# sandialabs/implicit-sph

Hardware: AMD Instinct MI355X
Metric: pressure-Poisson solves/sec (3D TGV, 1M particles per GPU, GMRES(50)+block-Jacobi ILU(0), tol 1e-8) (higher is better)
Workload: dtype f64; 1 GPU; 3D Taylor-Green vortex, 100^3 particles per GPU, Wendland cut=2h (BASELINE configs[1]), state after one Lagrangian step (mode=advect); rows_per_gpu=1000000, global_rows=1000000, nnz_per_gpu=103845090, solver=FGMRES(50) DGKS tol 1e-8, right prec, precond=bjacobi-ilu0, atom_order=lexicographic, library_row_order=bricks, parallelism=domain bricks 1x1x1, RCCL halo + all-reduce, restarts=1, converged=1

## Files before the change

### implicit-sph_amd/csrc/core.hpp

```cpp
#pragma once
#include "common.hpp"
#include "order.hpp"
#include "sell.hpp"

namespace isph { struct HostStager; }

struct isph_neigh_layout {
  const void *nptr = nullptr;
  const int *nidx = nullptr, *colmap = nullptr;
  const void *order = nullptr;
  int n = -1, is_sorted = 0;
  isph::DevBuf<long long> off;
  isph::DevBuf<int> idx, len, sorted;
  void release() { off.release(); idx.release(); len.release(); sorted.release(); nptr = nullptr; nidx = colmap = nullptr; order = nullptr; n = -1; is_sorted = 0; }
};

struct isph_neigh_map {
  const int *rowsrc = nullptr, *idmap = nullptr, *colmap_key = nullptr;
  const int *colkey = nullptr;
  const void *order = nullptr;
};

struct isph_table_cache {
  int ntypes = -1, kernel = -1, dim = -1;
  std::vector<int> kind;
  std::vector<double> h, cutsq;
  isph::DevBuf<int> dkind;
  isph::DevBuf<double> dh, dcutsq, dhinv, dknorm, dkdnorm;
  void release() { dkind.release(); dh.release(); dcutsq.release(); dhinv.release(); dknorm.release(); dkdnorm.release(); ntypes = -1; }
};

struct isph_ctx {
  int device = 0;
  hipStream_t stream = nullptr;
  bool own_stream = false;
  int rank = 0, nranks = 1;
  ncclComm_t comm = nullptr;
  isph_host_transport host_tr = {nullptr, nullptr, nullptr};
  double *hsend = nullptr, *hrecv = nullptr;
  size_t hsend_cap = 0, hrecv_cap = 0;
  bool profile = false;
  int stat_reorth = 0;
  isph::DevBuf<double> partial;
  isph::DevBuf<double> dscal;
  double *hscal = nullptr;
  size_t hscal_cap = 0;
  isph::DevBuf<double> V, Z, wv, tv, rv, pv, nvec, xext, sendbuf, bdev, xdev;
  isph::DevBuf<double> bint, xint;
  isph::DevBuf<int> imask, imask2;
  std::vector<hipEvent_t> ev;
  std::vector<int> ev_class;
  size_t ev_used = 0;
  std::vector<hipEvent_t> hev;
  size_t hev_used = 0;
  hipEvent_t ev0 = nullptr, ev1 = nullptr;
  hipEvent_t ev_fetch = nullptr;
  std::vector<hipEvent_t> ev_ls;
  hipStream_t comm_stream = nullptr;
  hipEvent_t ev_pack = nullptr, ev_halo = nullptr;
  isph::DevBuf<double> xghost;
  isph::HostStager *stager = nullptr;
  bool neigh_hold = false;
  isph_neigh_layout neigh_cache[2];
  isph_table_cache tables;
  int ordering = 1;
  isph::OrderBox box;
  isph_neigh_map nmap;
  isph::RowOrderPtr held_order;
  const void *held_key[2] = {nullptr, nullptr};
};

namespace isph {
enum ProfClass { PROF_SPMV = 0, PROF_PREC_APPLY, PROF_MULTI_DOT, PROF_MULTI_AXPY_DOT, PROF_MULTI_AXPY_NORM, PROF_ILU_EXTRACT,
                 PROF_ILU_SCHEDULE, PROF_ILU_FACTOR, PROF_NCLASS };
struct ProfScope {
  isph_ctx *c;
  size_t slot = (size_t)-1;
  ProfScope(isph_ctx *ctx, int cls, hipStream_t st = nullptr) : c(ctx) {
    if (!c || !c->profile || (st && st != c->stream)) return;
    if (c->ev_used + 2 > c->ev.size()) {
      hipEvent_t a = nullptr, b = nullptr;
      if (hipEventCreate(&a) != hipSuccess || hipEventCreate(&b) != hipSuccess) return;
      c->ev.push_back(a); c->ev.push_back(b);
      c->ev_class.push_back(cls);
    }
    slot = c->ev_used;
    c->ev_class[slot / 2] = cls;
    c->ev_used += 2;
    (void)hipEventRecord(c->ev[slot], c->stream);
  }
  ~ProfScope() { end(); }
  void end() {
    if (slot != (size_t)-1) (void)hipEventRecord(c->ev[slot + 1], c->stream);
    slot = (size_t)-1;
  }
};
}

// ... 40 lines not shown
```

### implicit-sph_amd/csrc/krylov.hpp

```cpp
#pragma once
#include "common.hpp"

namespace isph {

constexpr int kDotBatch = 16;

__global__ __launch_bounds__(kBlock) void k_multi_dot_v2(int n, int nk, const double *__restrict__ V, long long ld,
                                                         const double *__restrict__ w, double *__restrict__ partial) {
  __shared__ double sred[kDotBatch + 1][4];
  const int wave = threadIdx.x >> 6, lane = threadIdx.x & 63;
  const long long stride = (long long)gridDim.x * kBlock, np = n >> 1;
  const long long p0 = (long long)blockIdx.x * kBlock + threadIdx.x;
  const double2 *__restrict__ w2 = reinterpret_cast<const double2 *>(w);
  for (int k0 = 0; k0 < nk || k0 == 0; k0 += kDotBatch) {
    const int nb = min(kDotBatch, nk - k0);
    const bool last = k0 + kDotBatch >= nk;
    double acc[kDotBatch];
#pragma unroll
    for (int u = 0; u < kDotBatch; ++u) acc[u] = 0.0;
    double ww = 0.0;
    const double *__restrict__ vb = V + (long long)k0 * ld;
    for (long long p = p0; p < np; p += stride) {
      const double2 wi = w2[p];
      if (last) ww = fma(wi.y, wi.y, fma(wi.x, wi.x, ww));
// ... 69 lines not shown
#pragma unroll
      for (int u = 0; u < kDotBatch; ++u)
        if (u < nb) acc[u] = fma(vb[(long long)u * ld + i], wi, acc[u]);
    }
#pragma unroll
    for (int u = 0; u < kDotBatch; ++u) {
      if (u < nb) {
        const double s = wave_sum(acc[u]);
        if (lane == 0) sred[u][wave] = s;
      }
    }
    if (last) {
      ww = wave_sum(ww);
      if (lane == 0) sred[kDotBatch][wave] = ww;
    }
    __syncthreads();
    if (threadIdx.x < nb)
      partial[(long long)(k0 + threadIdx.x) * gridDim.x + blockIdx.x] =
          (sred[threadIdx.x][0] + sred[threadIdx.x][1]) + (sred[threadIdx.x][2] + sred[threadIdx.x][3]);
    if (last && threadIdx.x == 0)
      partial[(long long)nk * gridDim.x + blockIdx.x] =
          (sred[kDotBatch][0] + sred[kDotBatch][1]) + (sred[kDotBatch][2] + sred[kDotBatch][3]);
    __syncthreads();
    if (last) break;
  }
}

__global__ __launch_bounds__(kBlock) void k_reduce_partials(int nk, int nblk, const double *__restrict__ partial,
                                                            double *__restrict__ out,
                                                            const double *__restrict__ flag = nullptr) {
  __shared__ double sw[4];
  const int k = blockIdx.x;
  if (k >= nk) return;
  if (flag && *flag == 0.0) {
    if (threadIdx.x == 0) out[k] = 0.0;
    return;
  }
  const double *__restrict__ p = partial + (long long)k * nblk;
  double s0 = 0.0, s1 = 0.0, s2 = 0.0, s3 = 0.0;
  int b = threadIdx.x;
  for (; b + 3 * kBlock < nblk; b += 4 * kBlock) {
    s0 += p[b];
    s1 += p[b + kBlock];
    s2 += p[b + 2 * kBlock];
    s3 += p[b + 3 * kBlock];
  }
  for (; b < nblk; b += kBlock) s0 += p[b];
  double s = wave_sum((s0 + s1) + (s2 + s3));
  if ((threadIdx.x & 63) == 0) sw[threadIdx.x >> 6] = s;
  __syncthreads();
  if (threadIdx.x == 0) out[k] = (sw[0] + sw[1]) + (sw[2] + sw[3]);
}

__global__ __launch_bounds__(kBlock) void k_multi_axpy_norm(int n, int nk, const double *__restrict__ V, long long ld,
                                                            const double *__restrict__ c, double *__restrict__ w,
                                                            double *__restrict__ partial,
                                                            const double *__restrict__ dec_old = nullptr,
                                                            const double *__restrict__ dec_dn = nullptr, int dec_force = 0,
                                                            double *__restrict__ dec_out = nullptr,
                                                            double *__restrict__ vnext = nullptr) {
  __shared__ double sw[4];
  __shared__ double sdec[2];
  bool second = true;
  double wfinal2 = 1.0;
  if (dec_old) {
    if (threadIdx.x == 0) {
      double old2 = *dec_old;
      if (dec_dn) old2 = fmax(old2 - dec_dn[0] * dec_dn[0], 0.0);
      const double ww_new = c[nk];
      const bool sec = dec_force || sqrt(ww_new) < M_SQRT1_2 * sqrt(old2);
      double s2 = 0.0;
      for (int k = 0; k < nk; ++k) s2 += c[k] * c[k];
      sdec[0] = sec ? 1.0 : 0.0;
      sdec[1] = sec ? fmax(ww_new - s2, 0.0) : ww_new;
      if (blockIdx.x == 0) { dec_out[0] = sdec[0]; dec_out[1] = sdec[1]; }
    }
    __syncthreads();
    second = sdec[0] != 0.0;
    wfinal2 = sdec[1];
  }
  if (!second && !vnext) return;
  double a = 1.0;
  if (vnext) a *= 1.0 / sqrt(wfinal2);
  double ww = 0.0;
  for (long long i = (long long)blockIdx.x * blockDim.x + threadIdx.x; i < n; i += (long long)gridDim.x * blockDim.x) {
    double s = w[i];
    if (second) {
      for (int k = 0; k < nk; ++k) s = fma(-c[k], V[(long long)k * ld + i], s);
      w[i] = s;
    }
    if (vnext) vnext[i] = a * s;
    ww = fma(s, s, ww);
  }
  ww = wave_sum(ww);
  if ((threadIdx.x & 63) == 0) sw[threadIdx.x >> 6] = ww;
  __syncthreads();
  if (threadIdx.x == 0) partial[blockIdx.x] = (sw[0] + sw[1]) + (sw[2] + sw[3]);
}

template <int NK>
__global__ __launch_bounds__(kBlock) void k_multi_axpy_dot(int n, int nk, const double *__restrict__ V, long long ld,
                                                           const double *__restrict__ c, double *__restrict__ w,
                                                           double *__restrict__ partial) {
  __shared__ double sred[NK + 1][4];
  __shared__ double sc[NK];
  const int wave = threadIdx.x >> 6, lane = threadIdx.x & 63;
  if (threadIdx.x < NK) sc[threadIdx.x] = threadIdx.x < nk ? c[threadIdx.x] : 0.0;
  __syncthreads();
  double acc[NK];
#pragma unroll
  for (int u = 0; u < NK; ++u) acc[u] = 0.0;
  double ww = 0.0;
  const long long stride = (long long)gridDim.x * kBlock;
  for (long long i = (long long)blockIdx.x * kBlock + threadIdx.x; i < n; i += stride) {
    double v[NK];
#pragma unroll
    for (int u = 0; u < NK; ++u) v[u] = u < nk ? V[(long long)u * ld + i] : 0.0;
    double s = w[i];
#pragma unroll
    for (int u = 0; u < NK; ++u) s = fma(-sc[u], v[u], s);
    w[i] = s;
    ww = fma(s, s, ww);
#pragma unroll
    for (int u = 0; u < NK; ++u) acc[u] = fma(v[u], s, acc[u]);
  }
#pragma unroll
  for (int u = 0; u < NK; ++u) {
    if (u < nk) {
      const double r = wave_sum(acc[u]);
      if (lane == 0) sred[u][wave] = r;
    }
  }
  ww = wave_sum(ww);
  if (lane == 0) sred[NK][wave] = ww;
  __syncthreads();
  if (threadIdx.x < nk)
    partial[(long long)threadIdx.x * gridDim.x + blockIdx.x] =
        (sred[threadIdx.x][0] + sred[threadIdx.x][1]) + (sred[threadIdx.x][2] + sred[threadIdx.x][3]);
  if (threadIdx.x == 0)
    partial[(long long)nk * gridDim.x + blockIdx.x] = (sred[NK][0] + sred[NK][1]) + (sred[NK][2] + sred[NK][3]);
}

__global__ void k_multi_axpy(int n, int nk, const double *__restrict__ Z, long long ld, const double *__restrict__ c,
                             double *__restrict__ x) {
  for (long long i = (long long)blockIdx.x * blockDim.x + threadIdx.x; i < n; i += (long long)gridDim.x * blockDim.x) {
    double s = x[i];
    for (int k = 0; k < nk; ++k) s = fma(c[k], Z[(long long)k * ld + i], s);
    x[i] = s;
  }
}

__global__ __launch_bounds__(kBlock) void k_dot2(int n, const double *__restrict__ a, const double *__restrict__ b,
                                                 const double *__restrict__ c, const double *__restrict__ d,
                                                 double *__restrict__ partial) {
  __shared__ double s0[4], s1[4];
  double p = 0.0, q = 0.0;
  for (long long i = (long long)blockIdx.x * blockDim.x + threadIdx.x; i < n; i += (long long)gridDim.x * blockDim.x) {
    p = fma(a[i], b[i], p);
    if (c) q = fma(c[i], d[i], q);
  }
  p = wave_sum(p);
  q = wave_sum(q);
  if ((threadIdx.x & 63) == 0) { s0[threadIdx.x >> 6] = p; s1[threadIdx.x >> 6] = q; }
  __syncthreads();
  if (threadIdx.x == 0) {
    partial[blockIdx.x] = (s0[0] + s0[1]) + (s0[2] + s0[3]);
    partial[gridDim.x + blockIdx.x] = (s1[0] + s1[1]) + (s1[2] + s1[3]);
  }
}

__global__ void k_scale_copy(int n, const double *__restrict__ x, double *__restrict__ y, double alpha,
                             const double *__restrict__ s, int inv_sqrt) {
  double a = alpha;
  if (s) a *= inv_sqrt ? 1.0 / sqrt(*s) : *s;
  for (long long i = (long long)blockIdx.x * blockDim.x + threadIdx.x; i < n; i += (long long)gridDim.x * blockDim.x)
    y[i] = a * x[i];
}

__global__ void k_axpy_dev(int n, double alpha, const double *__restrict__ s, const double *__restrict__ x,
                           double *__restrict__ y) {
  const double a = s ? alpha * (*s) : alpha;
  for (long long i = (long long)blockIdx.x * blockDim.x + threadIdx.x; i < n; i += (long long)gridDim.x * blockDim.x)
    y[i] = fma(a, x[i], y[i]);
}

__global__ void k_residual(int n, const double *__restrict__ b, double *__restrict__ r) {
  for (long long i = (long long)blockIdx.x * blockDim.x + threadIdx.x; i < n; i += (long long)gridDim.x * blockDim.x)
    r[i] = b[i] - r[i];
}

__global__ void k_cg_update_p(int n, const double *__restrict__ z, double *__restrict__ p,
                              const double *__restrict__ num, const double *__restrict__ den) {
  const double beta = *num / *den;
  for (long long i = (long long)blockIdx.x * blockDim.x + threadIdx.x; i < n; i += (long long)gridDim.x * blockDim.x)
    p[i] = fma(beta, p[i], z[i]);
}

__global__ __launch_bounds__(kBlock) void k_cg_update_xr(int n, const double *__restrict__ p,
                                                         const double *__restrict__ ap, double *__restrict__ x,
                                                         double *__restrict__ r, const double *__restrict__ num,
                                                         const double *__restrict__ den, double *__restrict__ partial) {
  __shared__ double sw[4];
  const double a = *num / *den;
  double rr = 0.0;
  for (long long i = (long long)blockIdx.x * blockDim.x + threadIdx.x; i < n; i += (long long)gridDim.x * blockDim.x) {
    x[i] = fma(a, p[i], x[i]);
    const double t = fma(-a, ap[i], r[i]);
    r[i] = t;
    rr = fma(t, t, rr);
  }
  rr = wave_sum(rr);
  if ((threadIdx.x & 63) == 0) sw[threadIdx.x >> 6] = rr;
  __syncthreads();
  if (threadIdx.x == 0) partial[blockIdx.x] = (sw[0] + sw[1]) + (sw[2] + sw[3]);
}

__global__ void k_mul_elem(int n, const double *__restrict__ a, const double *__restrict__ b, double *__restrict__ y) {
  for (long long i = (long long)blockIdx.x * blockDim.x + threadIdx.x; i < n; i += (long long)gridDim.x * blockDim.x)
    y[i] = a[i] * b[i];
}

__global__ void k_fill(int n, double *__restrict__ y, double v) {
  for (long long i = (long long)blockIdx.x * blockDim.x + threadIdx.x; i < n; i += (long long)gridDim.x * blockDim.x)
    y[i] = v;
}

__global__ void k_mask_to_double(int n, const int *__restrict__ m, double *__restrict__ y) {
  for (long long i = (long long)blockIdx.x * blockDim.x + threadIdx.x; i < n; i += (long long)gridDim.x * blockDim.x)
    y[i] = (double)m[i];
}

inline int stream_grid(long long n) {
  long long g = (n + kBlock - 1) / kBlock;
  if (g > kMaxRedBlocks) g = kMaxRedBlocks;
  if (g < 1) g = 1;
  return (int)g;
}

}
```

### implicit-sph_amd/csrc/solver.hpp

```cpp
#pragma once
#include <cmath>

#include "comm.hpp"
#include "core.hpp"
#include "krylov.hpp"

namespace isph {

int prec_apply_dev(isph_ctx *ctx, const isph_prec *M, const double *r, double *z);
int prec_apply_multi_dev(isph_ctx *ctx, const isph_prec *M, int K, const double *const *rs, double *const *zs);

inline int allreduce_inplace(isph_ctx *ctx, double *d, int count) {
  return comm_allreduce(ctx, d, count,  0, ctx->stream);
}

enum { SC_DOT = 0 , SC_Y = 64 , SC_MISC = 128, SC_COUNT = 160 };

constexpr int kMaxLockstep = 4;

inline int ensure_scalars(isph_ctx *ctx) {
  ISPH_CHECK(ctx->dscal.reserve(SC_COUNT * kMaxLockstep));
  ISPH_CHECK(ctx->partial.reserve((size_t)kMaxRedBlocks * 66));
  if (ctx->hscal_cap < (size_t)SC_COUNT * kMaxLockstep) {
    if (ctx->hscal) (void)hipHostFree(ctx->hscal);
    ISPH_CHECK_HIP(hipHostMalloc((void **)&ctx->hscal, (size_t)SC_COUNT * kMaxLockstep * sizeof(double)));
    ctx->hscal_cap = (size_t)SC_COUNT * kMaxLockstep;
  }
  return ISPH_SUCCESS;
}

inline int fetch_scalars(isph_ctx *ctx, int first, int count) {
  ISPH_CHECK_HIP(hipMemcpyAsync(ctx->hscal + first, ctx->dscal.p + first, sizeof(double) * (size_t)count,
                                hipMemcpyDeviceToHost, ctx->stream));
  ISPH_CHECK_HIP(hipStreamSynchronize(ctx->stream));
  return ISPH_SUCCESS;
}

__global__ void k_gather(int n, const int *__restrict__ idx, const double *__restrict__ x, double *__restrict__ out) {
  for (int i = blockIdx.x * blockDim.x + threadIdx.x; i < n; i += gridDim.x * blockDim.x) out[i] = x[idx[i]];
}

inline int halo_begin(isph_ctx *ctx, const isph_mat *A, const double *x, hipEvent_t *hev = nullptr) {
  ISPH_REQUIRE(comm_active(ctx) && ctx->comm_stream,
               "a matrix with a halo needs a context made by isph_ctx_create_dist or isph_ctx_create_hostcomm");
  const Sell &S = A->S;
  const isph_halo &H = A->halo;
  ISPH_REQUIRE(H.nrecv == S.ncol - S.nrow, "matrix has ghost columns but no matching halo plan");
  ISPH_REQUIRE(H.n_int + H.n_bnd == S.nslices, "halo plan without the interior/boundary slice lists");
  ISPH_CHECK(ctx->xghost.reserve((size_t)(H.nrecv > 0 ? H.nrecv : 1)));
  ISPH_CHECK(ctx->sendbuf.reserve((size_t)(H.nsend > 0 ? H.nsend : 1)));
  if (H.nsend > 0)
    hipLaunchKernelGGL(k_gather, dim3(stream_grid(H.nsend)), dim3(kBlock), 0, ctx->stream, H.nsend, H.send_idx.p, x,
                       ctx->sendbuf.p);
  ISPH_CHECK_HIP(hipEventRecord(ctx->ev_pack, ctx->stream));
  if (hev) ISPH_CHECK_HIP(hipEventRecord(hev[0], ctx->stream));
  ISPH_CHECK_HIP(hipStreamWaitEvent(ctx->comm_stream, ctx->ev_pack, 0));
  ISPH_CHECK(comm_exchange(ctx, H, ctx->sendbuf.p, ctx->xghost.p, 1, false, ctx->comm_stream));
  ISPH_CHECK_HIP(hipEventRecord(ctx->ev_halo, ctx->comm_stream));
  if (hev) ISPH_CHECK_HIP(hipEventRecord(hev[1], ctx->comm_stream));
  return ISPH_SUCCESS;
}

inline bool sell_cols16(isph_ctx *ctx, const Sell &S) {
  if (S.c16_state != 0) return S.c16_state > 0;
  S.c16_state = -1;
  if (S.nslices == 0 || S.stored == 0) return false;
  DevTmp<int> flag;
  if (flag.reserve(1) != ISPH_SUCCESS || S.col16.reserve((size_t)S.stored) != ISPH_SUCCESS ||
      S.wtab.reserve((size_t)S.nslices * 64) != ISPH_SUCCESS) { flag.release(); return false; }
  int h = 0;
  if (hipMemsetAsync(flag.p, 0, sizeof(int), ctx->stream) == hipSuccess) {
    hipLaunchKernelGGL(k_sell_compress_cols, dim3((S.nslices + 3) / 4), dim3(kBlock), 0, ctx->stream, 0, S.nslices,
                       (const long long *)S.slice_off.p, (const int *)S.col.p, S.col16.p, S.wtab.p, flag.p);
    if (hipMemcpyAsync(&h, flag.p, sizeof(int), hipMemcpyDeviceToHost, ctx->stream) == hipSuccess &&
        hipStreamSynchronize(ctx->stream) == hipSuccess && hipGetLastError() == hipSuccess && h == 0)
      S.c16_state = 1;
  }
  flag.release();
// ... 111 lines not shown
          if (!first)
            hipLaunchKernelGGL(k_axpy_dev, dim3(stream_grid(nloc)), dim3(kBlock), 0, ctx->stream, nloc, 1.0,
                               (const double *)nullptr, (const double *)tmp, yi);
          first = false;
        }
        if (first) ISPH_CHECK_HIP(hipMemsetAsync(yi, 0, sizeof(double) * (size_t)nloc, ctx->stream));
      }
      return ISPH_SUCCESS;
    }
    ISPH_CHECK(spmv_dev(ctx, A, x, y, nvec));
    if (nvec)
      hipLaunchKernelGGL(k_axpy_dev, dim3(stream_grid(n)), dim3(kBlock), 0, ctx->stream, n, -1.0,
                         ctx->dscal.p + SC_MISC, nvec, y);
    return ISPH_SUCCESS;
  }
  int prec(const double *r, double *z) const {
    if (!M) {
      ISPH_CHECK_HIP(hipMemcpyAsync(z, r, sizeof(double) * (size_t)n, hipMemcpyDeviceToDevice, ctx->stream));
      return ISPH_SUCCESS;
    }
    if (blk) {
      const double *rs[4];
      double *zs[4];
      for (int i = 0; i < dim && i < 4; ++i) { rs[i] = r + (size_t)i * nloc; zs[i] = z + (size_t)i * nloc; }
      return prec_apply_multi_dev(ctx, M, dim, rs, zs);
    }
    return prec_apply_dev(ctx, M, r, z);
  }
};

inline int dot_dev(isph_ctx *ctx, int n, const double *a, const double *b, const double *c, const double *d, int slot) {
  const int g = stream_grid(n);
  hipLaunchKernelGGL(k_dot2, dim3(g), dim3(kBlock), 0, ctx->stream, n, a, b, c, d, ctx->partial.p);
  hipLaunchKernelGGL(k_reduce_partials, dim3(2), dim3(kBlock), 0, ctx->stream, 2, g, ctx->partial.p, ctx->dscal.p + slot);
  return allreduce_inplace(ctx, ctx->dscal.p + slot, 2);
}

inline int project_dev(isph_ctx *ctx, int n, const double *nvec, double *v) {
  ISPH_CHECK(dot_dev(ctx, n, v, nvec, nullptr, nullptr, SC_MISC + 2));
  hipLaunchKernelGGL(k_axpy_dev, dim3(stream_grid(n)), dim3(kBlock), 0, ctx->stream, n, -1.0, ctx->dscal.p + SC_MISC + 2,
                     nvec, v);
  return ISPH_SUCCESS;
}

inline int cgs_pass(isph_ctx *ctx, int n, int nk, const double *V, long long ld, double *w) {
  int g = stream_grid(n);
  if (g > 1024) g = 1024;
  ISPH_CHECK(ctx->partial.reserve((size_t)(nk + 2) * kMaxRedBlocks > (size_t)kMaxRedBlocks * 66 ? (size_t)(nk + 2) * kMaxRedBlocks : (size_t)kMaxRedBlocks * 66));
  hipLaunchKernelGGL((k_multi_dot<1>), dim3(g), dim3(kBlock), 0, ctx->stream, n, nk, V, ld, w, ctx->partial.p);
  hipLaunchKernelGGL(k_reduce_partials, dim3(nk + 1), dim3(kBlock), 0, ctx->stream, nk + 1, g, ctx->partial.p,
                     ctx->dscal.p + SC_DOT);
  ISPH_CHECK(allreduce_inplace(ctx, ctx->dscal.p + SC_DOT, nk + 1));
  const int g2 = stream_grid(n);
  hipLaunchKernelGGL(k_multi_axpy_norm, dim3(g2), dim3(kBlock), 0, ctx->stream, n, nk, V, ld, ctx->dscal.p + SC_DOT, w,
                     ctx->partial.p);
  hipLaunchKernelGGL(k_reduce_partials, dim3(1), dim3(kBlock), 0, ctx->stream, 1, g2, ctx->partial.p,
                     ctx->dscal.p + SC_DOT + nk + 1);
  ISPH_CHECK(allreduce_inplace(ctx, ctx->dscal.p + SC_DOT + nk + 1, 1));
  ISPH_CHECK_HIP(hipGetLastError());
  return fetch_scalars(ctx, SC_DOT, nk + 2);
}

enum { SC_ORTHO = SC_MISC + 20 };
inline int ortho_enqueue(isph_ctx *ctx, int n, int nk, const double *V, long long ld, double *w, int ortho, double *vnext,
                         bool deflate = false, int mb = 0) {
  int g = stream_grid(n);
  if (g > 1024) g = 1024;
  ISPH_CHECK(ctx->partial.reserve((size_t)kMaxRedBlocks * 66));
  hipStream_t st = ctx->stream;
  double *dh1 = ctx->dscal.p + mb + SC_DOT, *dh2 = ctx->dscal.p + mb + SC_Y, *dor = ctx->dscal.p + mb + SC_ORTHO;
  constexpr int dot_grid = 512;
  if (g > dot_grid) g = dot_grid;
  {
    ProfScope prof(ctx, PROF_MULTI_DOT);
    if ((reinterpret_cast<uintptr_t>(w) & 15) == 0 && (reinterpret_cast<uintptr_t>(V) & 15) == 0)
      hipLaunchKernelGGL(k_multi_dot_v2, dim3(g), dim3(kBlock), 0, st, n, nk, V, ld, w, ctx->partial.p);
    else
      hipLaunchKernelGGL((k_multi_dot<2>), dim3(g), dim3(kBlock), 0, st, n, nk, V, ld, w, ctx->partial.p);
  }
  hipLaunchKernelGGL(k_reduce_partials, dim3(nk + 1), dim3(kBlock), 0, st, nk + 1, g, ctx->partial.p, dh1,
                     (const double *)nullptr);
  ISPH_CHECK(allreduce_inplace(ctx, dh1, nk + 1));
  {
    ProfScope prof(ctx, PROF_MULTI_AXPY_DOT);
    if (nk <= 16)
      hipLaunchKernelGGL((k_multi_axpy_dot<16>), dim3(g), dim3(kBlock), 0, st, n, nk, V, ld, dh1, w, ctx->partial.p);
    else if (nk <= 32)
      hipLaunchKernelGGL((k_multi_axpy_dot<32>), dim3(g), dim3(kBlock), 0, st, n, nk, V, ld, dh1, w, ctx->partial.p);
    else if (nk <= 48)
      hipLaunchKernelGGL((k_multi_axpy_dot<48>), dim3(g), dim3(kBlock), 0, st, n, nk, V, ld, dh1, w, ctx->partial.p);
    else
      hipLaunchKernelGGL((k_multi_axpy_dot<64>), dim3(g), dim3(kBlock), 0, st, n, nk, V, ld, dh1, w, ctx->partial.p);
  }
  hipLaunchKernelGGL(k_reduce_partials, dim3(nk + 1), dim3(kBlock), 0, st, nk + 1, g, ctx->partial.p, dh2,
                     (const double *)nullptr);
  ISPH_CHECK(allreduce_inplace(ctx, dh2, nk + 1));
  const int g2 = stream_grid(n);
  {
    ProfScope prof(ctx, PROF_MULTI_AXPY_NORM);
    hipLaunchKernelGGL(k_multi_axpy_norm, dim3(g2), dim3(kBlock), 0, st, n, nk, V, ld, (const double *)dh2, w, ctx->partial.p,
                       (const double *)(dh1 + nk), deflate ? (const double *)dh1 : (const double *)nullptr, ortho == 1 ? 1 : 0,
                       dor, vnext);
  }
  ISPH_CHECK_HIP(hipGetLastError());
  return ISPH_SUCCESS;
}

inline void ortho_collect(isph_ctx *ctx, int nk, double *h, double *wnorm, int mb = 0) {
  const double *hs = ctx->hscal + mb;
  const bool second = hs[SC_ORTHO] != 0.0;
  if (second) ++ctx->stat_reorth;
  for (int k = 0; k < nk; ++k) h[k] = hs[SC_DOT + k] + (second ? hs[SC_Y + k] : 0.0);
  *wnorm = std::sqrt(hs[SC_ORTHO + 1]);
}

inline int orthogonalize(isph_ctx *ctx, int n, int j, const double *V, long long ld, double *w, double *h, int ortho,
                         double *wnorm) {
  const int nk = j + 1;
  for (int k = 0; k < nk; ++k) h[k] = 0.0;
  if (ortho == 2) {
    double nn = 0.0;
    for (int pass = 0; pass < 2; ++pass)
      for (int k = 0; k < nk; ++k) {
        ISPH_CHECK(cgs_pass(ctx, n, 1, V + (long long)k * ld, ld, w));
        h[k] += ctx->hscal[SC_DOT];
        nn = ctx->hscal[SC_DOT + 2];
      }
    *wnorm = std::sqrt(nn);
    return ISPH_SUCCESS;
  }
  ISPH_CHECK(ortho_enqueue(ctx, n, nk, V, ld, w, ortho, nullptr));
  ISPH_CHECK(fetch_scalars(ctx, 0, SC_COUNT));
  ortho_collect(ctx, nk, h, wnorm);
  return ISPH_SUCCESS;
}

inline int gmres(const LinOp &op, const double *b, double *x, const isph_solver_params *prm, isph_solve_info *info) {
  isph_ctx *ctx = op.ctx;
  const int n = op.n, m = prm->num_blocks;
  ISPH_REQUIRE(m >= 1 && m <= 62, "Num Blocks must be in [1,62]");
  const long long ld = ((long long)n + 63) / 64 * 64;
  const bool deflate = op.nvec != nullptr && !op.blk && prm->ortho != 2;
  ISPH_CHECK(ctx->V.reserve((size_t)ld * (size_t)(m + 2)));
  if (prm->flexible) ISPH_CHECK(ctx->Z.reserve((size_t)ld * (size_t)m));
  ISPH_CHECK(ctx->wv.reserve((size_t)ld));
  ISPH_CHECK(ctx->tv.reserve((size_t)ld));
  double *Vall = ctx->V.p, *V = ctx->V.p + (deflate ? ld : 0), *Z = ctx->Z.p, *w = ctx->wv.p, *t = ctx->tv.p;
  if (deflate)
    ISPH_CHECK_HIP(hipMemcpyAsync(Vall, op.nvec, sizeof(double) * (size_t)n, hipMemcpyDeviceToDevice, ctx->stream));
  std::vector<double> H((size_t)(m + 1) * (size_t)m, 0.0), cs((size_t)m), sn((size_t)m), g((size_t)m + 1), y((size_t)m);
  const int sg = stream_grid(n);
  hipStream_t st = ctx->stream;

  ISPH_CHECK(op.apply(x, w));
  hipLaunchKernelGGL(k_residual, dim3(sg), dim3(kBlock), 0, st, n, b, w);
  ISPH_CHECK(dot_dev(ctx, n, w, w, nullptr, nullptr, SC_MISC + 4));
  ISPH_CHECK(fetch_scalars(ctx, SC_MISC + 4, 1));
  double beta = std::sqrt(ctx->hscal[SC_MISC + 4]);
  const double scale = beta == 0.0 ? 1.0 : beta;
  info->iters = 0;
  info->restarts = 0;
  info->converged = 0;
  info->rel_res_implicit = beta / scale;
  if (beta / scale <= prm->tol) info->converged = 1;

  while (!info->converged && info->iters < prm->max_iters) {
    hipLaunchKernelGGL(k_scale_copy, dim3(sg), dim3(kBlock), 0, st, n, w, V, 1.0 / beta, (const double *)nullptr, 0);
    std::fill(g.begin(), g.end(), 0.0);
    g[0] = beta;
    int j = 0;
    auto enqueue_op = [&](int col) -> int {
      const double *zj;
      double *vj = V + (long long)col * ld;
      if (prm->flexible) {
        ISPH_CHECK(op.prec(vj, Z + (long long)col * ld));
        zj = Z + (long long)col * ld;
      } else {
        ISPH_CHECK(op.prec(vj, t));
        zj = t;
      }
      return deflate ? spmv_dev(ctx, op.A, zj, w, nullptr) : op.apply(zj, w);
    };
    bool op_queued = false;
    while (j < m) {
      if (!op_queued) ISPH_CHECK(enqueue_op(j));
      op_queued = false;
      double *h = &H[(size_t)j * (size_t)(m + 1)];
      double wn = 0.0;
      if (prm->ortho == 2) {
        ISPH_CHECK(orthogonalize(ctx, n, j, V, ld, w, h, prm->ortho, &wn));
        if (wn != 0.0)
          hipLaunchKernelGGL(k_scale_copy, dim3(sg), dim3(kBlock), 0, st, n, w, V + (long long)(j + 1) * ld, 1.0 / wn,
                             (const double *)nullptr, 0);
      } else {
        const int nkt = j + 1 + (deflate ? 1 : 0);
        ISPH_CHECK(ortho_enqueue(ctx, n, nkt, Vall, ld, w, prm->ortho, V + (long long)(j + 1) * ld, deflate));
        ISPH_CHECK_HIP(hipMemcpyAsync(ctx->hscal, ctx->dscal.p, sizeof(double) * SC_COUNT, hipMemcpyDeviceToHost, st));
        ISPH_CHECK_HIP(hipEventRecord(ctx->ev_fetch, st));
        if (j + 1 < m && info->iters + 1 < prm->max_iters) {
          ISPH_CHECK(enqueue_op(j + 1));
          op_queued = true;
        }
        ISPH_CHECK_HIP(hipEventSynchronize(ctx->ev_fetch));
        if (deflate) {
          double hh[66];
          ortho_collect(ctx, nkt, hh, &wn);
          for (int k = 0; k <= j; ++k) h[k] = hh[k + 1];
        } else {
          ortho_collect(ctx, nkt, h, &wn);
        }
      }
      h[j + 1] = wn;
      for (int k = 0; k < j; ++k) {
        const double a = cs[k] * h[k] + sn[k] * h[k + 1];
        h[k + 1] = -sn[k] * h[k] + cs[k] * h[k + 1];
        h[k] = a;
      }
      {
        const double a = h[j], bb = h[j + 1], rr = std::hypot(a, bb);
        cs[j] = rr == 0.0 ? 1.0 : a / rr;
        sn[j] = rr == 0.0 ? 0.0 : bb / rr;
        h[j] = rr;
        h[j + 1] = 0.0;
        g[j + 1] = -sn[j] * g[j];
        g[j] = cs[j] * g[j];
      }
      ++j;
      ++info->iters;
      info->rel_res_implicit = std::fabs(g[j]) / scale;
      if (prm->verbose && ctx->rank == 0 && info->iters % 10 == 0)
        printf(">> isph::gmres iter %d  rel res %.3e\n", info->iters, info->rel_res_implicit);
      if (info->rel_res_implicit <= prm->tol) { info->converged = 1; break; }
      if (info->iters >= prm->max_iters) break;
    }
    for (int k = j - 1; k >= 0; --k) {
      double s = g[k];
      for (int l = k + 1; l < j; ++l) s -= H[(size_t)l * (size_t)(m + 1) + k] * y[l];
      y[k] = s / H[(size_t)k * (size_t)(m + 1) + k];
    }
    for (int k = 0; k < j; ++k) ctx->hscal[SC_Y + k] = y[k];
    ISPH_CHECK_HIP(hipMemcpyAsync(ctx->dscal.p + SC_Y, ctx->hscal + SC_Y, sizeof(double) * (size_t)j, hipMemcpyHostToDevice, st));
    if (prm->flexible) {
      hipLaunchKernelGGL(k_multi_axpy, dim3(sg), dim3(kBlock), 0, st, n, j, Z, ld, ctx->dscal.p + SC_Y, x);
    } else {
      hipLaunchKernelGGL(k_fill, dim3(sg), dim3(kBlock), 0, st, n, w, 0.0);
      hipLaunchKernelGGL(k_multi_axpy, dim3(sg), dim3(kBlock), 0, st, n, j, V, ld, ctx->dscal.p + SC_Y, w);
      ISPH_CHECK(op.prec(w, t));
      hipLaunchKernelGGL(k_axpy_dev, dim3(sg), dim3(kBlock), 0, st, n, 1.0, (const double *)nullptr, t, x);
    }
    ISPH_CHECK_HIP(hipStreamSynchronize(st));
    if (info->converged || info->iters >= prm->max_iters) break;
    if (info->restarts >= prm->max_restarts) break;
    ++info->restarts;
    ISPH_CHECK(op.apply(x, w));
    hipLaunchKernelGGL(k_residual, dim3(sg), dim3(kBlock), 0, st, n, b, w);
    ISPH_CHECK(dot_dev(ctx, n, w, w, nullptr, nullptr, SC_MISC + 4));
    ISPH_CHECK(fetch_scalars(ctx, SC_MISC + 4, 1));
    beta = std::sqrt(ctx->hscal[SC_MISC + 4]);
    if (beta == 0.0) { info->converged = 1; break; }
  }
  ISPH_CHECK_HIP(hipGetLastError());
  return ISPH_SUCCESS;
}

inline bool gmres_lockstep_ok(const LinOp &op, const isph_solver_params *prm, int K) {
  return K >= 2 && K <= kMaxLockstep && !op.nvec && !op.blk && prm->flexible && prm->ortho != 2 && prm->solver_type == 0;
}

inline int gmres_lockstep(const LinOp &op, int K, const double *const *bs, double *const *xs, const isph_solver_params *prm,
                          isph_solve_info *infos) {
  isph_ctx *ctx = op.ctx;
  const int n = op.n, m = prm->num_blocks;
  ISPH_REQUIRE(m >= 1 && m <= 62, "Num Blocks must be in [1,62]");
  const long long ld = ((long long)n + 63) / 64 * 64;
  ISPH_CHECK(ctx->V.reserve((size_t)ld * (size_t)(m + 2) * (size_t)K));
  ISPH_CHECK(ctx->Z.reserve((size_t)ld * (size_t)m * (size_t)K));
  ISPH_CHECK(ctx->wv.reserve((size_t)ld * (size_t)K));
  while ((int)ctx->ev_ls.size() < K) {
    hipEvent_t e;
    ISPH_CHECK_HIP(hipEventCreateWithFlags(&e, hipEventDisableTiming));
    ctx->ev_ls.push_back(e);
  }
  struct Sys {
    double *V, *Z, *w;
    std::vector<double> H, cs, sn, g, y;
    double beta = 0.0, scale = 1.0;
    int j = 0;
    bool in_cycle = false, done = false;
  };
  std::vector<Sys> sys((size_t)K);
  const int sg = stream_grid(n);
  hipStream_t st = ctx->stream;
  const double *xin[kMaxLockstep];
  double *yout[kMaxLockstep];
  for (int k = 0; k < K; ++k) {
    Sys &s = sys[(size_t)k];
    s.V = ctx->V.p + (size_t)k * ld * (size_t)(m + 2);
    s.Z = ctx->Z.p + (size_t)k * ld * (size_t)m;
    s.w = ctx->wv.p + (size_t)k * ld;
    s.H.assign((size_t)(m + 1) * (size_t)m, 0.0);
    s.cs.assign((size_t)m, 0.0); s.sn.assign((size_t)m, 0.0); s.g.assign((size_t)m + 1, 0.0); s.y.assign((size_t)m, 0.0);
    infos[k].iters = 0; infos[k].restarts = 0; infos[k].converged = 0;
    xin[k] = xs[k]; yout[k] = s.w;
  }
  ISPH_CHECK(spmm_dev(ctx, op.A, K, xin, yout));
  for (int k = 0; k < K; ++k) {
    Sys &s = sys[(size_t)k];
    hipLaunchKernelGGL(k_residual, dim3(sg), dim3(kBlock), 0, st, n, bs[k], s.w);
    ISPH_CHECK(dot_dev(ctx, n, s.w, s.w, nullptr, nullptr, SC_MISC + 4));
    ISPH_CHECK(fetch_scalars(ctx, SC_MISC + 4, 1));
    s.beta = std::sqrt(ctx->hscal[SC_MISC + 4]);
    s.scale = s.beta == 0.0 ? 1.0 : s.beta;
    infos[k].rel_res_implicit = s.beta / s.scale;
    if (s.beta / s.scale <= prm->tol) { infos[k].converged = 1; s.done = true; }
  }
  auto start_cycle = [&](int k) {
    Sys &s = sys[(size_t)k];
    hipLaunchKernelGGL(k_scale_copy, dim3(sg), dim3(kBlock), 0, st, n, s.w, s.V, 1.0 / s.beta, (const double *)nullptr, 0);
    std::fill(s.g.begin(), s.g.end(), 0.0);
    s.g[0] = s.beta;
    s.j = 0;
    s.in_cycle = true;
  };
  auto end_cycle = [&](int k) -> int {
    Sys &s = sys[(size_t)k];
    isph_solve_info &inf = infos[k];
    const int j = s.j, mb = k * SC_COUNT;
    for (int q = j - 1; q >= 0; --q) {
      double acc = s.g[(size_t)q];
      for (int l = q + 1; l < j; ++l) acc -= s.H[(size_t)l * (size_t)(m + 1) + q] * s.y[(size_t)l];
      s.y[(size_t)q] = acc / s.H[(size_t)q * (size_t)(m + 1) + q];
    }
    for (int q = 0; q < j; ++q) ctx->hscal[mb + SC_Y + q] = s.y[(size_t)q];
    ISPH_CHECK_HIP(hipMemcpyAsync(ctx->dscal.p + mb + SC_Y, ctx->hscal + mb + SC_Y, sizeof(double) * (size_t)j, hipMemcpyHostToDevice, st));
    hipLaunchKernelGGL(k_multi_axpy, dim3(sg), dim3(kBlock), 0, st, n, j, s.Z, ld, ctx->dscal.p + mb + SC_Y, xs[k]);
    ISPH_CHECK_HIP(hipStreamSynchronize(st));
    s.in_cycle = false;
    if (inf.converged || inf.iters >= prm->max_iters || inf.restarts >= prm->max_restarts) { s.done = true; return ISPH_SUCCESS; }
    ++inf.restarts;
    ISPH_CHECK(op.apply(xs[k], s.w));
    hipLaunchKernelGGL(k_residual, dim3(sg), dim3(kBlock), 0, st, n, bs[k], s.w);
    ISPH_CHECK(dot_dev(ctx, n, s.w, s.w, nullptr, nullptr, SC_MISC + 4));
    ISPH_CHECK(fetch_scalars(ctx, SC_MISC + 4, 1));
    s.beta = std::sqrt(ctx->hscal[SC_MISC + 4]);
    if (s.beta == 0.0) { inf.converged = 1; s.done = true; return ISPH_SUCCESS; }
    start_cycle(k);
    return ISPH_SUCCESS;
  };
  for (int k = 0; k < K; ++k)
    if (!sys[(size_t)k].done) {
      if (infos[k].iters < prm->max_iters) start_cycle(k);
      else sys[(size_t)k].done = true;
    }
  int act[kMaxLockstep];
  while (true) {
    int na = 0;
    for (int k = 0; k < K; ++k)
      if (!sys[(size_t)k].done && sys[(size_t)k].in_cycle) act[na++] = k;
    if (na == 0) break;
    {
      const double *vin[kMaxLockstep];
      double *zout[kMaxLockstep];
      for (int a = 0; a < na; ++a) {
        Sys &s = sys[(size_t)act[a]];
        vin[a] = s.V + (long long)s.j * ld;
        zout[a] = s.Z + (long long)s.j * ld;
        xin[a] = zout[a];
        yout[a] = s.w;
      }
      if (op.M) ISPH_CHECK(prec_apply_multi_dev(ctx, op.M, na, vin, zout));
      else
        for (int a = 0; a < na; ++a) ISPH_CHECK(op.prec(vin[a], zout[a]));
    }
    ISPH_CHECK(spmm_dev(ctx, op.A, na, xin, yout));
    for (int a = 0; a < na; ++a) {
      const int k = act[a], mb = k * SC_COUNT;
      Sys &s = sys[(size_t)k];
      ISPH_CHECK(ortho_enqueue(ctx, n, s.j + 1, s.V, ld, s.w, prm->ortho, s.V + (long long)(s.j + 1) * ld, false, mb));
      ISPH_CHECK_HIP(hipMemcpyAsync(ctx->hscal + mb, ctx->dscal.p + mb, sizeof(double) * SC_COUNT, hipMemcpyDeviceToHost, st));
      ISPH_CHECK_HIP(hipEventRecord(ctx->ev_ls[(size_t)k], st));
    }
    for (int a = 0; a < na; ++a) {
      const int k = act[a], mb = k * SC_COUNT;
      Sys &s = sys[(size_t)k];
      isph_solve_info &inf = infos[k];
      ISPH_CHECK_HIP(hipEventSynchronize(ctx->ev_ls[(size_t)k]));
      const int j = s.j;
      double *h = &s.H[(size_t)j * (size_t)(m + 1)];
      double wn = 0.0;
      for (int q = 0; q <= j; ++q) h[q] = 0.0;
      ortho_collect(ctx, j + 1, h, &wn, mb);
      h[j + 1] = wn;
      for (int q = 0; q < j; ++q) {
        const double t = s.cs[(size_t)q] * h[q] + s.sn[(size_t)q] * h[q + 1];
        h[q + 1] = -s.sn[(size_t)q] * h[q] + s.cs[(size_t)q] * h[q + 1];
        h[q] = t;
      }
      {
        const double t = h[j], bb = h[j + 1], rr = std::hypot(t, bb);
        s.cs[(size_t)j] = rr == 0.0 ? 1.0 : t / rr;
        s.sn[(size_t)j] = rr == 0.0 ? 0.0 : bb / rr;
        h[j] = rr;
        h[j + 1] = 0.0;
        s.g[(size_t)j + 1] = -s.sn[(size_t)j] * s.g[(size_t)j];
        s.g[(size_t)j] = s.cs[(size_t)j] * s.g[(size_t)j];
      }
      ++s.j;
      ++inf.iters;
      inf.rel_res_implicit = std::fabs(s.g[(size_t)s.j]) / s.scale;
      if (prm->verbose && ctx->rank == 0 && inf.iters % 10 == 0)
        printf(">> isph::gmres[%d] iter %d  rel res %.3e\n", k, inf.iters, inf.rel_res_implicit);
      if (inf.rel_res_implicit <= prm->tol) inf.converged = 1;
      if (inf.converged || inf.iters >= prm->max_iters || s.j >= m) ISPH_CHECK(end_cycle(k));
    }
  }
  ISPH_CHECK_HIP(hipGetLastError());
  return ISPH_SUCCESS;
}

inline int pcg(const LinOp &op, const double *b, double *x, const isph_solver_params *prm, isph_solve_info *info) {
  isph_ctx *ctx = op.ctx;
  const int n = op.n;
  const long long ld = ((long long)n + 63) / 64 * 64;
  ISPH_CHECK(ctx->wv.reserve((size_t)ld));
  ISPH_CHECK(ctx->tv.reserve((size_t)ld));
  ISPH_CHECK(ctx->rv.reserve((size_t)ld));
  ISPH_CHECK(ctx->pv.reserve((size_t)ld));
  double *r = ctx->rv.p, *z = ctx->tv.p, *p = ctx->pv.p, *ap = ctx->wv.p;
  const int sg = stream_grid(n);
  hipStream_t st = ctx->stream;
  double *ds = ctx->dscal.p;
  enum { RZ = SC_MISC + 8, PAP = SC_MISC + 10, RR = SC_MISC + 12, RZN = SC_MISC + 14 };
// ... 48 lines not shown
```

Before: 25.40 solves/s (1M-particle bricks; x n_gpus under weak scaling).

## Fuse GMRES ortho reductions into consumer kernels and mail scalars to pinned host

On single-rank runs, the separate partial-reduction kernels after the multi-dot and multi-axpy-dot steps are folded into the following kernels, which each reduce the block partials locally. The final ortho kernel writes its scalars straight into coherent pinned host memory, so the device-to-host copy is no longer needed. The change also skips queuing the next operator when the residual trend predicts convergence, and skips the initial SpMV when x0 is all zeros. The aim is fewer launches and syncs per Arnoldi step, at the cost of every block redundantly reducing the partials and an extra zero check with a host sync at solve start.

```diff
diff --git a/implicit-sph_amd/csrc/core.hpp b/implicit-sph_amd/csrc/core.hpp
--- a/implicit-sph_amd/csrc/core.hpp
+++ b/implicit-sph_amd/csrc/core.hpp
@@ -44,6 +44,8 @@
   isph::DevBuf<double> partial;
   isph::DevBuf<double> dscal;
   double *hscal = nullptr;
+  double *hscal_dev = nullptr;
+  int step_norm_grid = 1024;
   size_t hscal_cap = 0;
   isph::DevBuf<double> V, Z, wv, tv, rv, pv, nvec, xext, sendbuf, bdev, xdev;
   isph::DevBuf<double> bint, xint;
diff --git a/implicit-sph_amd/csrc/krylov.hpp b/implicit-sph_amd/csrc/krylov.hpp
--- a/implicit-sph_amd/csrc/krylov.hpp
+++ b/implicit-sph_amd/csrc/krylov.hpp
@@ -145,15 +145,57 @@
   if (threadIdx.x == 0) out[k] = (sw[0] + sw[1]) + (sw[2] + sw[3]);
 }
 
+template <int B>
+__device__ __forceinline__ void wg_reduce_partials(int ncol, int nblk, const double *__restrict__ partial, double (*sred)[4]) {
+  const int wave = threadIdx.x >> 6, lane = threadIdx.x & 63;
+  const int b0 = threadIdx.x, b1 = threadIdx.x + kBlock;
+  for (int k0 = 0; k0 < ncol; k0 += B) {
+    double v0[B], v1[B];
+#pragma unroll
+    for (int u = 0; u < B; ++u) {
+      const double *__restrict__ p = partial + (long long)min(k0 + u, ncol - 1) * nblk;
+      v0[u] = b0 < nblk ? p[b0] : 0.0;
+      v1[u] = b1 < nblk ? p[b1] : 0.0;
+    }
+#pragma unroll
+    for (int u = 0; u < B; ++u) {
+      const double r = wave_sum((0.0 + v0[u]) + v1[u]);
+      if (lane == 0 && k0 + u < ncol) sred[k0 + u][wave] = r;
+    }
+  }
+  __syncthreads();
+}
+__device__ __forceinline__ double red_combine(const double *sw) { return (sw[0] + sw[1]) + (sw[2] + sw[3]); }
+
+struct StepMail {
+  const double *c1 = nullptr;
+  double *dot = nullptr, *y = nullptr, *dec = nullptr;
+};
+template <bool RED>
 __global__ __launch_bounds__(kBlock) void k_multi_axpy_norm(int n, int nk, const double *__restrict__ V, long long ld,
-                                                            const double *__restrict__ c, double *__restrict__ w,
+                                                            const double *__restrict__ c_in, double *__restrict__ w,
                                                             double *__restrict__ partial,
                                                             const double *__restrict__ dec_old = nullptr,
                                                             const double *__restrict__ dec_dn = nullptr, int dec_force = 0,
                                                             double *__restrict__ dec_out = nullptr,
-                                                            double *__restrict__ vnext = nullptr) {
+                                                            double *__restrict__ vnext = nullptr,
+                                                            const double *__restrict__ red_in = nullptr, int red_g = 0,
+                                                            double *__restrict__ c_out = nullptr, StepMail mail = StepMail()) {
   __shared__ double sw[4];
   __shared__ double sdec[2];
+  __shared__ double sc2[RED ? 65 : 1];
+  __shared__ double sredn[RED ? 65 : 1][4];
+  const double *__restrict__ c = c_in;
+  if (RED) {
+    wg_reduce_partials<12>(nk + 1, red_g, red_in, sredn);
+    if (threadIdx.x <= nk) {
+      const double v = red_combine(sredn[threadIdx.x]);
+      sc2[threadIdx.x] = v;
+      if (blockIdx.x == 0) c_out[threadIdx.x] = v;
+    }
+    __syncthreads();
+    c = sc2;
+  }
   bool second = true;
   double wfinal2 = 1.0;
   if (dec_old) {
@@ -171,6 +213,11 @@
     __syncthreads();
     second = sdec[0] != 0.0;
     wfinal2 = sdec[1];
+    if (mail.dot && blockIdx.x == 0) {
+      if (threadIdx.x <= nk) { mail.dot[threadIdx.x] = mail.c1[threadIdx.x]; mail.y[threadIdx.x] = c[threadIdx.x]; }
+      if (threadIdx.x == 0) { mail.dec[0] = sdec[0]; mail.dec[1] = sdec[1]; }
+      __threadfence_system();
+    }
   }
   if (!second && !vnext) return;
   double a = 1.0;
@@ -194,11 +241,19 @@
 template <int NK>
 __global__ __launch_bounds__(kBlock) void k_multi_axpy_dot(int n, int nk, const double *__restrict__ V, long long ld,
                                                            const double *__restrict__ c, double *__restrict__ w,
-                                                           double *__restrict__ partial) {
+                                                           double *__restrict__ partial,
+                                                           const double *__restrict__ red_in = nullptr, int red_g = 0,
+                                                           double *__restrict__ c_out = nullptr) {
   __shared__ double sred[NK + 1][4];
   __shared__ double sc[NK];
   const int wave = threadIdx.x >> 6, lane = threadIdx.x & 63;
-  if (threadIdx.x < NK) sc[threadIdx.x] = threadIdx.x < nk ? c[threadIdx.x] : 0.0;
+  if (red_in) {
+    wg_reduce_partials<16>(nk + 1, red_g, red_in, sred);
+    if (threadIdx.x < NK) sc[threadIdx.x] = threadIdx.x < nk ? red_combine(sred[threadIdx.x]) : 0.0;
+    if (blockIdx.x == 0 && threadIdx.x <= nk) c_out[threadIdx.x] = red_combine(sred[threadIdx.x]);
+  } else {
+    if (threadIdx.x < NK) sc[threadIdx.x] = threadIdx.x < nk ? c[threadIdx.x] : 0.0;
+  }
   __syncthreads();
   double acc[NK];
 #pragma unroll
@@ -280,6 +335,14 @@
 __global__ void k_residual(int n, const double *__restrict__ b, double *__restrict__ r) {
   for (long long i = (long long)blockIdx.x * blockDim.x + threadIdx.x; i < n; i += (long long)gridDim.x * blockDim.x)
     r[i] = b[i] - r[i];
+}
+
+__global__ __launch_bounds__(kBlock) void k_nonzero_partials(int n, const double *__restrict__ x, double *__restrict__ partial) {
+  int any = 0;
+  for (long long i = (long long)blockIdx.x * blockDim.x + threadIdx.x; i < n; i += (long long)gridDim.x * blockDim.x)
+    any |= (((unsigned long long)__double_as_longlong(x[i])) << 1) != 0ull;
+  any = __syncthreads_or(any);
+  if (threadIdx.x == 0) partial[blockIdx.x] = any ? 1.0 : 0.0;
 }
 
 __global__ void k_cg_update_p(int n, const double *__restrict__ z, double *__restrict__ p,
diff --git a/implicit-sph_amd/csrc/solver.hpp b/implicit-sph_amd/csrc/solver.hpp
--- a/implicit-sph_amd/csrc/solver.hpp
+++ b/implicit-sph_amd/csrc/solver.hpp
@@ -1,5 +1,7 @@
 #pragma once
 #include <cmath>
+#include <cstdlib>
+#include <cstring>
 
 #include "comm.hpp"
 #include "core.hpp"
@@ -18,12 +20,17 @@
 
 constexpr int kMaxLockstep = 4;
 
+constexpr size_t kPartialRegion = (size_t)kMaxRedBlocks * 66;
+constexpr size_t kPartialDoubles = 2 * kPartialRegion + (size_t)kMaxRedBlocks;
+
 inline int ensure_scalars(isph_ctx *ctx) {
   ISPH_CHECK(ctx->dscal.reserve(SC_COUNT * kMaxLockstep));
-  ISPH_CHECK(ctx->partial.reserve((size_t)kMaxRedBlocks * 66));
+  ISPH_CHECK(ctx->partial.reserve(kPartialDoubles));
   if (ctx->hscal_cap < (size_t)SC_COUNT * kMaxLockstep) {
     if (ctx->hscal) (void)hipHostFree(ctx->hscal);
-    ISPH_CHECK_HIP(hipHostMalloc((void **)&ctx->hscal, (size_t)SC_COUNT * kMaxLockstep * sizeof(double)));
+    ctx->hscal = nullptr; ctx->hscal_dev = nullptr; ctx->hscal_cap = 0;
+    ISPH_CHECK_HIP(hipHostMalloc((void **)&ctx->hscal, (size_t)SC_COUNT * kMaxLockstep * sizeof(double), hipHostMallocCoherent));
+    ISPH_CHECK_HIP(hipHostGetDevicePointer((void **)&ctx->hscal_dev, ctx->hscal, 0));
     ctx->hscal_cap = (size_t)SC_COUNT * kMaxLockstep;
   }
   return ISPH_SUCCESS;
@@ -241,8 +248,8 @@
                      ctx->dscal.p + SC_DOT);
   ISPH_CHECK(allreduce_inplace(ctx, ctx->dscal.p + SC_DOT, nk + 1));
   const int g2 = stream_grid(n);
-  hipLaunchKernelGGL(k_multi_axpy_norm, dim3(g2), dim3(kBlock), 0, ctx->stream, n, nk, V, ld, ctx->dscal.p + SC_DOT, w,
-                     ctx->partial.p);
+  hipLaunchKernelGGL((k_multi_axpy_norm<false>), dim3(g2), dim3(kBlock), 0, ctx->stream, n, nk, V, ld,
+                     (const double *)(ctx->dscal.p + SC_DOT), w, ctx->partial.p);
   hipLaunchKernelGGL(k_reduce_partials, dim3(1), dim3(kBlock), 0, ctx->stream, 1, g2, ctx->partial.p,
                      ctx->dscal.p + SC_DOT + nk + 1);
   ISPH_CHECK(allreduce_inplace(ctx, ctx->dscal.p + SC_DOT + nk + 1, 1));
@@ -251,45 +258,92 @@
 }
 
 enum { SC_ORTHO = SC_MISC + 20 };
+
+enum {
+  STEP_RED1 = 1,
+  STEP_RED2 = 2,
+  STEP_MAIL = 4,
+  STEP_PREDICT = 8,
+  STEP_ZERO_X0 = 16,
+  STEP_DEFAULT = STEP_RED1 | STEP_RED2 | STEP_MAIL | STEP_PREDICT | STEP_ZERO_X0
+};
+constexpr int kNormGridFused = 1024;
+inline unsigned gmres_step_parts(isph_ctx *ctx) {
+  ctx->step_norm_grid = kNormGridFused;
+  if (ctx->nranks > 1) return 0;
+  if (const char *ng = getenv("ISPH_GMRES_NORM_GRID")) {
+    const int v = atoi(ng);
+    if (v >= 1 && v <= kMaxRedBlocks) ctx->step_norm_grid = v;
+  }
+  const char *leg = getenv("ISPH_GMRES_LEGACY_STEP");
+  if (leg && leg[0] == '1') return 0;
+  const char *sel = getenv("ISPH_GMRES_STEP_PARTS");
+  if (!sel) return STEP_DEFAULT;
+  unsigned parts = 0;
+  if (strstr(sel, "1a")) parts |= STEP_RED1;
+  if (strstr(sel, "1b")) parts |= STEP_RED2;
+  if (strchr(sel, '2')) parts |= STEP_MAIL;
+  if (strchr(sel, '3')) parts |= STEP_PREDICT;
+  if (strchr(sel, '4')) parts |= STEP_ZERO_X0;
+  return parts;
+}
+
 inline int ortho_enqueue(isph_ctx *ctx, int n, int nk, const double *V, long long ld, double *w, int ortho, double *vnext,
-                         bool deflate = false, int mb = 0) {
+                         bool deflate = false, int mb = 0, unsigned parts = 0) {
   int g = stream_grid(n);
   if (g > 1024) g = 1024;
-  ISPH_CHECK(ctx->partial.reserve((size_t)kMaxRedBlocks * 66));
+  ISPH_CHECK(ctx->partial.reserve(kPartialDoubles));
   hipStream_t st = ctx->stream;
+  double *const part1 = ctx->partial.p, *const part2 = parts ? part1 + kPartialRegion : part1,
+               *const part3 = parts ? part1 + 2 * kPartialRegion : part1;
+  const bool red1 = parts & STEP_RED1, red2 = parts & STEP_RED2;
   double *dh1 = ctx->dscal.p + mb + SC_DOT, *dh2 = ctx->dscal.p + mb + SC_Y, *dor = ctx->dscal.p + mb + SC_ORTHO;
   constexpr int dot_grid = 512;
   if (g > dot_grid) g = dot_grid;
   {
     ProfScope prof(ctx, PROF_MULTI_DOT);
     if ((reinterpret_cast<uintptr_t>(w) & 15) == 0 && (reinterpret_cast<uintptr_t>(V) & 15) == 0)
-      hipLaunchKernelGGL(k_multi_dot_v2, dim3(g), dim3(kBlock), 0, st, n, nk, V, ld, w, ctx->partial.p);
+      hipLaunchKernelGGL(k_multi_dot_v2, dim3(g), dim3(kBlock), 0, st, n, nk, V, ld, w, part1);
     else
-      hipLaunchKernelGGL((k_multi_dot<2>), dim3(g), dim3(kBlock), 0, st, n, nk, V, ld, w, ctx->partial.p);
-  }
-  hipLaunchKernelGGL(k_reduce_partials, dim3(nk + 1), dim3(kBlock), 0, st, nk + 1, g, ctx->partial.p, dh1,
-                     (const double *)nullptr);
-  ISPH_CHECK(allreduce_inplace(ctx, dh1, nk + 1));
+      hipLaunchKernelGGL((k_multi_dot<2>), dim3(g), dim3(kBlock), 0, st, n, nk, V, ld, w, part1);
+  }
+  if (!red1) {
+    hipLaunchKernelGGL(k_reduce_partials, dim3(nk + 1), dim3(kBlock), 0, st, nk + 1, g, part1, dh1, (const double *)nullptr);
+    ISPH_CHECK(allreduce_inplace(ctx, dh1, nk + 1));
+  }
   {
     ProfScope prof(ctx, PROF_MULTI_AXPY_DOT);
+    const double *rin = red1 ? part1 : nullptr;
     if (nk <= 16)
-      hipLaunchKernelGGL((k_multi_axpy_dot<16>), dim3(g), dim3(kBlock), 0, st, n, nk, V, ld, dh1, w, ctx->partial.p);
+      hipLaunchKernelGGL((k_multi_axpy_dot<16>), dim3(g), dim3(kBlock), 0, st, n, nk, V, ld, dh1, w, part2, rin, g, dh1);
     else if (nk <= 32)
-      hipLaunchKernelGGL((k_multi_axpy_dot<32>), dim3(g), dim3(kBlock), 0, st, n, nk, V, ld, dh1, w, ctx->partial.p);
+      hipLaunchKernelGGL((k_multi_axpy_dot<32>), dim3(g), dim3(kBlock), 0, st, n, nk, V, ld, dh1, w, part2, rin, g, dh1);
     else if (nk <= 48)
-      hipLaunchKernelGGL((k_multi_axpy_dot<48>), dim3(g), dim3(kBlock), 0, st, n, nk, V, ld, dh1, w, ctx->partial.p);
+      hipLaunchKernelGGL((k_multi_axpy_dot<48>), dim3(g), dim3(kBlock), 0, st, n, nk, V, ld, dh1, w, part2, rin, g, dh1);
     else
-      hipLaunchKernelGGL((k_multi_axpy_dot<64>), dim3(g), dim3(kBlock), 0, st, n, nk, V, ld, dh1, w, ctx->partial.p);
-  }
-  hipLaunchKernelGGL(k_reduce_partials, dim3(nk + 1), dim3(kBlock), 0, st, nk + 1, g, ctx->partial.p, dh2,
-                     (const double *)nullptr);
-  ISPH_CHECK(allreduce_inplace(ctx, dh2, nk + 1));
-  const int g2 = stream_grid(n);
+      hipLaunchKernelGGL((k_multi_axpy_dot<64>), dim3(g), dim3(kBlock), 0, st, n, nk, V, ld, dh1, w, part2, rin, g, dh1);
+  }
+  if (!red2) {
+    hipLaunchKernelGGL(k_reduce_partials, dim3(nk + 1), dim3(kBlock), 0, st, nk + 1, g, part2, dh2, (const double *)nullptr);
+    ISPH_CHECK(allreduce_inplace(ctx, dh2, nk + 1));
+  }
+  int g2 = stream_grid(n);
+  if (red2 && g2 > ctx->step_norm_grid) g2 = ctx->step_norm_grid;
+  StepMail mail;
+  if (parts & STEP_MAIL) {
+    double *hm = ctx->hscal_dev + mb;
+    mail.c1 = dh1; mail.dot = hm + SC_DOT; mail.y = hm + SC_Y; mail.dec = hm + SC_ORTHO;
+  }
   {
     ProfScope prof(ctx, PROF_MULTI_AXPY_NORM);
-    hipLaunchKernelGGL(k_multi_axpy_norm, dim3(g2), dim3(kBlock), 0, st, n, nk, V, ld, (const double *)dh2, w, ctx->partial.p,
-                       (const double *)(dh1 + nk), deflate ? (const double *)dh1 : (const double *)nullptr, ortho == 1 ? 1 : 0,
-                       dor, vnext);
+    if (red2)
+      hipLaunchKernelGGL((k_multi_axpy_norm<true>), dim3(g2), dim3(kBlock), 0, st, n, nk, V, ld, (const double *)dh2, w, part3,
+                         (const double *)(dh1 + nk), deflate ? (const double *)dh1 : (const double *)nullptr, ortho == 1 ? 1 : 0,
+                         dor, vnext, (const double *)part2, g, dh2, mail);
+    else
+      hipLaunchKernelGGL((k_multi_axpy_norm<false>), dim3(g2), dim3(kBlock), 0, st, n, nk, V, ld, (const double *)dh2, w, part3,
+                         (const double *)(dh1 + nk), deflate ? (const double *)dh1 : (const double *)nullptr, ortho == 1 ? 1 : 0,
+                         dor, vnext, (const double *)nullptr, 0, (double *)nullptr, mail);
   }
   ISPH_CHECK_HIP(hipGetLastError());
   return ISPH_SUCCESS;
@@ -341,8 +395,22 @@
   const int sg = stream_grid(n);
   hipStream_t st = ctx->stream;
 
-  ISPH_CHECK(op.apply(x, w));
-  hipLaunchKernelGGL(k_residual, dim3(sg), dim3(kBlock), 0, st, n, b, w);
+  const unsigned parts = gmres_step_parts(ctx);
+
+  bool x_zero = false;
+  if ((parts & STEP_ZERO_X0) && n > 0) {
+    hipLaunchKernelGGL(k_nonzero_partials, dim3(sg), dim3(kBlock), 0, st, n, (const double *)x, ctx->partial.p);
+    hipLaunchKernelGGL(k_reduce_partials, dim3(1), dim3(kBlock), 0, st, 1, sg, (const double *)ctx->partial.p,
+                       ctx->dscal.p + SC_MISC + 5, (const double *)nullptr);
+    ISPH_CHECK(fetch_scalars(ctx, SC_MISC + 5, 1));
+    x_zero = ctx->hscal[SC_MISC + 5] == 0.0;
+  }
+  if (x_zero) {
+    ISPH_CHECK_HIP(hipMemcpyAsync(w, b, sizeof(double) * (size_t)n, hipMemcpyDeviceToDevice, st));
+  } else {
+    ISPH_CHECK(op.apply(x, w));
+    hipLaunchKernelGGL(k_residual, dim3(sg), dim3(kBlock), 0, st, n, b, w);
+  }
   ISPH_CHECK(dot_dev(ctx, n, w, w, nullptr, nullptr, SC_MISC + 4));
   ISPH_CHECK(fetch_scalars(ctx, SC_MISC + 4, 1));
   double beta = std::sqrt(ctx->hscal[SC_MISC + 4]);
@@ -352,6 +420,7 @@
   info->converged = 0;
   info->rel_res_implicit = beta / scale;
   if (beta / scale <= prm->tol) info->converged = 1;
+  double res_prev = beta / scale, res_prev2 = -1.0;
 
   while (!info->converged && info->iters < prm->max_iters) {
     hipLaunchKernelGGL(k_scale_copy, dim3(sg), dim3(kBlock), 0, st, n, w, V, 1.0 / beta, (const double *)nullptr, 0);
@@ -383,10 +452,12 @@
                              (const double *)nullptr, 0);
       } else {
         const int nkt = j + 1 + (deflate ? 1 : 0);
-        ISPH_CHECK(ortho_enqueue(ctx, n, nkt, Vall, ld, w, prm->ortho, V + (long long)(j + 1) * ld, deflate));
-        ISPH_CHECK_HIP(hipMemcpyAsync(ctx->hscal, ctx->dscal.p, sizeof(double) * SC_COUNT, hipMemcpyDeviceToHost, st));
+        ISPH_CHECK(ortho_enqueue(ctx, n, nkt, Vall, ld, w, prm->ortho, V + (long long)(j + 1) * ld, deflate, 0, parts));
+        if (!(parts & STEP_MAIL))
+          ISPH_CHECK_HIP(hipMemcpyAsync(ctx->hscal, ctx->dscal.p, sizeof(double) * SC_COUNT, hipMemcpyDeviceToHost, st));
         ISPH_CHECK_HIP(hipEventRecord(ctx->ev_fetch, st));
-        if (j + 1 < m && info->iters + 1 < prm->max_iters) {
+        const bool last_foreseen = (parts & STEP_PREDICT) && res_prev2 > 0.0 && res_prev * (res_prev / res_prev2) <= prm->tol;
+        if (j + 1 < m && info->iters + 1 < prm->max_iters && !last_foreseen) {
           ISPH_CHECK(enqueue_op(j + 1));
           op_queued = true;
         }
@@ -417,6 +488,8 @@
       ++j;
       ++info->iters;
       info->rel_res_implicit = std::fabs(g[j]) / scale;
+      res_prev2 = res_prev;
+      res_prev = info->rel_res_implicit;
       if (prm->verbose && ctx->rank == 0 && info->iters % 10 == 0)
         printf(">> isph::gmres iter %d  rel res %.3e\n", info->iters, info->rel_res_implicit);
       if (info->rel_res_implicit <= prm->tol) { info->converged = 1; break; }
@@ -480,6 +553,7 @@
   std::vector<Sys> sys((size_t)K);
   const int sg = stream_grid(n);
   hipStream_t st = ctx->stream;
+  const unsigned parts = gmres_step_parts(ctx);
   const double *xin[kMaxLockstep];
   double *yout[kMaxLockstep];
   for (int k = 0; k < K; ++k) {
@@ -565,8 +639,9 @@
     for (int a = 0; a < na; ++a) {
       const int k = act[a], mb = k * SC_COUNT;
       Sys &s = sys[(size_t)k];
-      ISPH_CHECK(ortho_enqueue(ctx, n, s.j + 1, s.V, ld, s.w, prm->ortho, s.V + (long long)(s.j + 1) * ld, false, mb));
-      ISPH_CHECK_HIP(hipMemcpyAsync(ctx->hscal + mb, ctx->dscal.p + mb, sizeof(double) * SC_COUNT, hipMemcpyDeviceToHost, st));
+      ISPH_CHECK(ortho_enqueue(ctx, n, s.j + 1, s.V, ld, s.w, prm->ortho, s.V + (long long)(s.j + 1) * ld, false, mb, parts));
+      if (!(parts & STEP_MAIL))
+        ISPH_CHECK_HIP(hipMemcpyAsync(ctx->hscal + mb, ctx->dscal.p + mb, sizeof(double) * SC_COUNT, hipMemcpyDeviceToHost, st));
       ISPH_CHECK_HIP(hipEventRecord(ctx->ev_ls[(size_t)k], st));
     }
     for (int a = 0; a < na; ++a) {
```

New measurement: 24.86 solves/s (1M-particle bricks; x n_gpus under weak scaling). 0.978x the previous value.
